# ZhenlongYuan/TSAR-MVS

Measured on AMD Instinct MI355X. Metric: depthmap Mpixels/sec (ETH3D full-res, 8 iters), higher is better.
Workload: dtype f32

## Files before the change

include/tsar.h:

```cpp
#ifndef TSAR_H_
#define TSAR_H_

#include <stddef.h>
#include <stdint.h>

#ifdef __cplusplus
extern "C" {
#endif

#define TSAR_MAX_VIEWS 64
#define TSAR_MAXCOST 2.0f

#define TSAR_OK 0
#define TSAR_ERR_INVALID (-1)
#define TSAR_ERR_HIP (-2)
#define TSAR_ERR_STATE (-3)
#define TSAR_ERR_NOMEM (-4)

#define TSAR_MEM_HOST 0
#define TSAR_MEM_DEVICE 1

#define TSAR_COMB_ALL 0
#define TSAR_COMB_BEST_N 1
#define TSAR_COMB_ANGLE 2
// ... 196 lines not shown
void tsar_device_free(int device, void* p);
int tsar_device_write(int device, void* dst, const void* host_src, size_t bytes);
int tsar_peer_copy(int dst_device, void* dst, int src_device, const void* src, size_t bytes);

int tsar_enable_kernel_timing(tsar_ctx* ctx, int enable);
int tsar_reset_kernel_timing(tsar_ctx* ctx);
int tsar_get_kernel_timing(tsar_ctx* ctx, tsar_kernel_timing* out, int cap, int* n_out);

int tsar_selftest_sqrt(tsar_ctx* ctx, int mode, uint64_t seed, uint64_t* mismatches_out);
int tsar_selftest_divide(tsar_ctx* ctx, const float* X, const float* Y, const float* Z, size_t n, float* u_out, float* v_out, int ieee);
int tsar_selftest_divide_random(tsar_ctx* ctx, int log2_triples, uint64_t seed, int mode, int guarded, uint64_t* mismatches_out,
                                uint64_t* outside_guard_out);
int tsar_selftest_sweep_census(tsar_ctx* ctx, int colour, uint64_t* out8);
int tsar_selftest_sweep_repeat(tsar_ctx* ctx, int colour, void* memo_dev, uint64_t* out8);
int tsar_selftest_prune_census(tsar_ctx* ctx, int on, uint32_t* out32);
int tsar_selftest_slic_stage(tsar_ctx* ctx, int stage, int w, int h, int mw, int mh, const tsar_slic_settings* s, const void* in0,
                             const void* in1, void* inout);

#ifdef __cplusplus
}
#endif
#endif
```

tsar-mvs_amd/api.py:

```python
from __future__ import annotations

import ctypes as C
import os

import numpy as np

_HERE = os.path.dirname(os.path.abspath(__file__))
LIB_PATH = os.environ.get("TSAR_LIB") or os.path.join(_HERE, "libtsar_hip.so")

TSAR_OK = 0
TSAR_ERR_INVALID, TSAR_ERR_HIP, TSAR_ERR_STATE, TSAR_ERR_NOMEM = -1, -2, -3, -4
MEM_HOST, MEM_DEVICE = 0, 1
COMB_ALL, COMB_BEST_N, COMB_ANGLE, COMB_GOOD = 0, 1, 2, 3
FLAG_FIX_DOWN_FAR_SEED, FLAG_FIX_RIGHT_FAR_CMP, FLAG_STRICT_DIV = 1, 2, 4
FLAG_FIX_PLANE_FIT = 8
FLAG_NO_LINE_CLOSING = 16
FLAG_TEX_FILTER_8BIT = 32
FLAG_FIX_INIT_RADIUS = 64
MAXCOST = 2.0
MAX_VIEWS = 64


class TsarError(RuntimeError):
    def __init__(self, code, msg):
# ... 57 lines not shown
    "tsar_pm_init", "tsar_pm_iterate", "tsar_pm_iterate_final", "tsar_pm_sweep", "tsar_set_sweep_counter", "tsar_pm_cost_planes", "tsar_set_plane", "tsar_get_plane",
    "tsar_load_planes", "tsar_compute_disp", "tsar_compute_disp_final", "tsar_depth_to_plane", "tsar_get_result",
    "tsar_pyramid_views", "tsar_upsample_planes", "tsar_compute_disp_final_upsampled", "tsar_get_view_image",
    "tsar_set_geom_depths", "tsar_clear_geom", "tsar_pm_rescore", "tsar_get_geom_matrices",
    "tsar_geom_pyramid", "tsar_pyramid_planes", "tsar_upsample_merge",
    "tsar_default_geom_check_params", "tsar_geom_check",
    "tsar_default_geom_reproject_params", "tsar_geom_reproject", "tsar_pm_merge_depths",
    "tsar_default_plane_prior_params", "tsar_set_plane_prior", "tsar_clear_plane_prior", "tsar_get_plane_prior",
    "tsar_default_plane_prior_build_params", "tsar_build_plane_prior",
    "tsar_set_reliable_mask", "tsar_get_reliable_mask", "tsar_lrdiff", "tsar_getview", "tsar_wmf", "tsar_set_regions", "tsar_detect_weak_texture", "tsar_ransac_regions",
    "tsar_set_region_planes", "tsar_fake_depth", "tsar_fill_textureless",
    "tsar_default_slic_settings", "tsar_slic", "tsar_default_fusion_params", "tsar_fuse", "tsar_fuse_ctx",
    "tsar_default_cloud_distance_params", "tsar_cloud_distance_ctx", "tsar_cloud_distance",
    "tsar_default_cloud_voxels_params", "tsar_cloud_voxels_ctx", "tsar_cloud_voxels",
    "tsar_host_alloc", "tsar_host_free", "tsar_device_alloc", "tsar_device_free", "tsar_device_write", "tsar_peer_copy", "tsar_enable_kernel_timing", "tsar_reset_kernel_timing", "tsar_get_kernel_timing",
    "tsar_selftest_divide", "tsar_selftest_divide_random", "tsar_selftest_sqrt", "tsar_selftest_sweep_census", "tsar_selftest_prune_census", "tsar_selftest_sweep_repeat", "tsar_selftest_slic_stage",
]

_lib = None


def load_library(path: str = LIB_PATH):
    global _lib
    if _lib is not None:
        return _lib
    if not os.path.exists(path):
        raise ImportError(f"{path} not found: build it with `make -C tsar-mvs_amd/csrc` "
                          "(or __graft_entry__.build()); there is no CPU fallback")
    L = C.CDLL(path)
    L.tsar_last_error.restype = C.c_char_p
    L.tsar_last_error.argtypes = [C.c_void_p]
# ... 84 lines not shown
    if hasattr(L, "tsar_cloud_voxels_ctx"):
        L.tsar_default_cloud_voxels_params.restype = None
        L.tsar_default_cloud_voxels_params.argtypes = [C.POINTER(CloudVoxelsParams)]
        L.tsar_cloud_voxels.argtypes = [C.c_int, C.c_void_p, C.c_int64, C.c_int, C.POINTER(CloudVoxelsParams), C.c_void_p, C.c_int, C.c_void_p, C.c_void_p, C.c_int64,
                                        C.c_void_p, C.c_void_p, C.c_void_p, C.POINTER(C.c_int64), C.POINTER(C.c_int64), C.c_int]
        L.tsar_cloud_voxels_ctx.argtypes = [C.c_void_p] + list(L.tsar_cloud_voxels.argtypes[1:])
    L.tsar_get_stream.argtypes = [C.c_void_p, C.POINTER(C.c_void_p)]
    L.tsar_synchronize.argtypes = [C.c_void_p]
    L.tsar_enable_kernel_timing.argtypes = [C.c_void_p, C.c_int]
    L.tsar_reset_kernel_timing.argtypes = [C.c_void_p]
    L.tsar_get_kernel_timing.argtypes = [C.c_void_p, C.POINTER(KernelTiming), C.c_int, C.POINTER(C.c_int)]
    L.tsar_selftest_divide.argtypes = [C.c_void_p, C.c_void_p, C.c_void_p, C.c_void_p, C.c_size_t, C.c_void_p, C.c_void_p, C.c_int]
    L.tsar_selftest_sweep_census.argtypes = [C.c_void_p, C.c_int, C.POINTER(C.c_uint64)]
    if hasattr(L, "tsar_selftest_prune_census"):
        L.tsar_selftest_prune_census.argtypes = [C.c_void_p, C.c_int, C.POINTER(C.c_uint32)]
    L.tsar_selftest_sweep_repeat.argtypes = [C.c_void_p, C.c_int, C.c_void_p, C.POINTER(C.c_uint64)]
    L.tsar_selftest_sqrt.argtypes = [C.c_void_p, C.c_int, C.c_uint64, C.POINTER(C.c_uint64)]
    L.tsar_selftest_divide_random.argtypes = [C.c_void_p, C.c_int, C.c_uint64, C.c_int, C.c_int, C.POINTER(C.c_uint64), C.POINTER(C.c_uint64)]
    L.tsar_selftest_slic_stage.argtypes = [C.c_void_p, C.c_int, C.c_int, C.c_int, C.c_int, C.c_int, C.POINTER(SlicSettings), C.c_void_p, C.c_void_p, C.c_void_p]
    _lib = L
    return L


def default_params(**kw) -> Params:
    p = Params()
    load_library().tsar_default_params(C.byref(p))
    for k, v in kw.items():
        setattr(p, k, v)
    return p

# ... 346 lines not shown
        return bad.value

    def selftest_sweep_census(self, colour: int) -> dict:
        out = (C.c_uint64 * 8)()
        self._chk(self.L.tsar_selftest_sweep_census(self._ctx, colour, out))
        keys = ("waves", "arms_any_lane", "max_lane_survivors", "max_lane_survivors_nodup", "lane_survivors", "lane_survivors_nodup", "pixels", "arms_present")
        return dict(zip(keys, [int(v) for v in out]))

    def selftest_prune_census(self, on: bool):
        if on:
            self._chk(self.L.tsar_selftest_prune_census(self._ctx, 1, None))
            return None
        out = (C.c_uint32 * 32)()
        self._chk(self.L.tsar_selftest_prune_census(self._ctx, 0, out))
        return np.array(out, np.int64).reshape(8, 4)

    def selftest_divide_random(self, log2_triples: int, seed: int, mode: int, guarded: bool = True):
        bad, out = C.c_uint64(0), C.c_uint64(0)
        self._chk(self.L.tsar_selftest_divide_random(self._ctx, log2_triples, seed, mode, int(guarded), C.byref(bad), C.byref(out)))
        return bad.value, out.value

    def _slic_stage(self, stage, w, h, mw, mh, settings, in0, in1, inout):
        p1 = _ptr(in1)[0] if in1 is not None else None
        self._chk(self.L.tsar_selftest_slic_stage(self._ctx, stage, w, h, mw, mh, C.byref(settings), _ptr(in0)[0], p1, _ptr(inout)[0]))
        return inout

    def slic_convert(self, bgra, color_space=0):
        img = np.ascontiguousarray(bgra, np.uint8).reshape(-1, 4)
        return self._slic_stage(0, img.shape[0], 1, 0, 0, SlicSettings(20, 0, 5.0, 0, color_space), img, None, np.zeros((img.shape[0], 4), np.float32))

# ... 484 lines not shown
```

tsar-mvs_amd/csrc/pm_core.h:

```cpp
#pragma once
#include <type_traits>

#include "tsar_device_math.h"

#define PM_BLOCK 256
#define PM_RW 32

#include "pm_tap_common.h"

template <bool QUAD, bool DIFF = false>
DEVFN float sample_bilinear(const DevView& vw, int w, int h, int qpitch, float u, float v, bool q8 = false) {
    u = fminf(fmaxf(u, -1.0f), (float)w);
    v = fminf(fmaxf(v, -1.0f), (float)h);
    const float fu = floorf(u), fv = floorf(v);
    float ax = u - fu, ay = v - fv;
    if (q8) { ax = rintf(ax * 256.0f) * 0.00390625f; ay = rintf(ay * 256.0f) * 0.00390625f; }
    const int iu = (int)fu, iv = (int)fv;
    float t00, t10, t01, t11;
    if (QUAD) {
        const uint32_t off = (uint32_t)(__mul24(iv + 1, qpitch) + iu + 1) * 4u;
        const uint32_t q = *(global_u32_ptr)((const char __attribute__((address_space(1)))*)vw.quad + off);
        t00 = (float)(q & 0xffu);
        t10 = (float)((q >> 8) & 0xffu);
        t01 = (float)((q >> 16) & 0xffu);
// ... 132 lines not shown
    if (pp == nullptr) return c;
    typedef float prior_entry __attribute__((ext_vector_type(4)));
    const prior_entry q = ((const __attribute__((address_space(1))) prior_entry*)pp)[y * sc->w + x];
    const float Dp = q.w;
    const float a = fabsf(D - Dp);
    const float rel = a / Dp;
    const float dclip = sc->prior_depth_clip, nclip = sc->prior_normal_clip;
    const float r_d = rel < dclip ? rel / dclip : 1.0f;
    const float s = 1.0f - ((n4.x * q.x + n4.y * q.y) + n4.z * q.z);
    const float s0 = s < 0.0f ? 0.0f : s;
    const float r_n = s < nclip ? s0 / nclip : 1.0f;
    const float t = (sc->prior_weight_depth * r_d) + (sc->prior_weight_normal * r_n);
    return Dp > 0.0f ? c + t : c;
}

template <int NB, int HR, bool STRICT, bool QUAD, int V = 0, int BLK = PM_BLOCK>
DEVFN float multiview_cost(const DevScene* __restrict__ sc, const typename TileOf<QUAD>::type* tile, int tw, int own, const float* wts, const PixelRef& pr,
                           int x, int y, const float4& n4, int& beview, float& ratio, bool prune = false, float cost_now = 0.0f, int* skipped = nullptr) {
    constexpr bool GEOM = (V & TSAR_V_GEOM) != 0;
    constexpr bool PRUNE = (V & TSAR_V_PRUNE) != 0;
    static_assert(!PRUNE || !GEOM, "the bound speaks of the photometric cost alone");
    constexpr bool PAIR = (V & TSAR_V_PAIR) != 0;
    static_assert(!PAIR || (!PRUNE && !GEOM), "the paired gathers exist for the plain fast box-11 kernels");
    constexpr int VT = V & ~(TSAR_V_GEOM | TSAR_V_REDRAW | TSAR_V_PRUNE | TSAR_V_PAIR);
    float best[NB];
#pragma unroll
    for (int k = 0; k < NB; k++) best[k] = __builtin_inff();
    const int num = sc->n_sel;
    int valid = 0, bv = -1;
    float cmin = __builtin_inff();
    float depth_h = 0.0f;
    if constexpr (GEOM) depth_h = plane_depth(sc->ref, n4, x, y);
    int vi_next = sc->sel[0];
    for (int i = 0; i < num; i++) {
        const int vi = vi_next;
        vi_next = sc->sel[i + 1 < num ? i + 1 : i];
        float c;
        if constexpr ((VT & TSAR_V_LUT) != 0) c = view_cost_lut<STRICT, (VT >> 11) & 7, (VT & TSAR_V_BUF) != 0 && !STRICT, (VT & TSAR_V_MIX) != 0 && !STRICT>(sc, sc->view[vi], tile, tw, own, wts, pr, x, y, n4);
        else if constexpr (QUAD && HR == 5 && r5_production_variant(VT) && PRUNE) {
            static_assert((VT & 250) == 250 && !STRICT, "pruning instantiations exist for the fast row-wise loop");
            ViewPrune vp;
            vp.on = prune; vp.skipped = false;
            vp.cost_now = cmin < cost_now ? TSAR_MAXCOST : cost_now;
            c = view_cost_r5<false, true, true, (VT & TSAR_V_BUF) != 0, (VT & TSAR_V_MIX) != 0, BLK, 0, true>(sc, sc->view[vi], tile, tw, own, wts, pr, x, y, n4, &vp);
            if (vp.skipped) *skipped += 1;
        } else if constexpr (QUAD && HR == 5 && PAIR && VT == 250) {
            static_assert(!STRICT, "the paired gathers exist for the fast row-wise loop");
            c = view_cost_r5<false, true, true, false, false, BLK, 0, false, true>(sc, sc->view[vi], tile, tw, own, wts, pr, x, y, n4);
        } else if constexpr (QUAD && HR == 5 && r5_production_variant(VT))
            c = view_cost_r5<STRICT, (VT & 128) != 0 && !STRICT, (VT & 8) != 0, (VT & TSAR_V_BUF) != 0, (VT & TSAR_V_MIX) != 0, BLK>(sc, sc->view[vi], tile, tw, own, wts, pr, x, y, n4);
#ifdef TSAR_EXPERIMENTS
        else if constexpr (QUAD && HR == 5 && PAIR && VT == (250 | 4194304))
            c = view_cost_r5<false, true, true, false, false, BLK, 3, false, true>(sc, sc->view[vi], tile, tw, own, wts, pr, x, y, n4);
        else if constexpr (QUAD && HR == 5 && r5_diag_variant(VT))
            c = view_cost_r5<false, true, true, true, true, BLK, (VT & 4194304) ? 1 : 2>(sc, sc->view[vi], tile, tw, own, wts, pr, x, y, n4);
#endif
        else {
            static_assert(VT == 0, "unknown tap-loop variant");
            c = view_cost_generic<HR, STRICT, QUAD, BLK>(sc, sc->view[vi], tile, tw, own, wts, pr, x, y, n4);
        }
// ... 3 lines not shown
        valid -= (int32_t)__float_as_uint(c - TSAR_MAXCOST) >> 31;
        if constexpr (GEOM) c = c + geom_term(sc, sc->view[vi], vi, x, y, depth_h);
        {
            const uint32_t worse = (uint32_t)((int32_t)__float_as_uint(cmin - c) >> 31);
            asm("v_bfi_b32 %0, %1, %2, %3" : "=v"(bv) : "v"(worse), "v"(bv), "s"(vi));
            cmin = vmin(cmin, c);
        }
        float v = c;
#pragma unroll
        for (int k = 0; k < NB; k++) {
            const float lo = vmin(best[k], v), hi = vmax(best[k], v);
            best[k] = lo;
            v = hi;
        }
    }
    int nb = valid;
    if (sc->cost_comb == TSAR_COMB_BEST_N) nb = min(nb, sc->n_best);
    if (nb <= 0) { beview = -1; ratio = 0.f; return TSAR_MAXCOST; }
    float cost = 0.f;
#pragma unroll
    for (int k = 0; k < NB; k++)
        if (k < nb) cost += best[k];
    cost = cost / (float)nb;
    ratio = num >= 2 ? best[0] / best[1] : 0.f;
    beview = bv;
    if constexpr (GEOM) cost = add_prior_term(sc, x, y, n4, depth_h, cost);
    return cost;
}

DEVFN void strip_tile(int t, int tiles_x, int tiles_y, int sw, int& tx, int& ty) {
// ... 20 lines not shown
```

tsar-mvs_amd/csrc/pm_sweep_impl.h:

```cpp
#pragma once
#include "pm_dispatch.h"

#define SWEEP_SMALL_IMAGE_TILES 3072

#define CAND_SAME (1 << 30)

DEVFN void select_candidates(const DevScene* __restrict__ sc, const float* __restrict__ c_same, const float* __restrict__ c_other,
                             int x, int y, int cand[8]) {
    const int col = sc->w, row = sc->h;
    const int p = y * col + x;
    const bool fix_seed = sc->flags & TSAR_FLAG_FIX_DOWN_FAR_SEED, fix_cmp = sc->flags & TSAR_FLAG_FIX_RIGHT_FAR_CMP;
    float cmin;
    int cp, cs;
#pragma unroll
    for (int k = 0; k < 8; k++) cand[k] = -1;
    if (y > 2) {
        cp = p - 3 * col; cmin = c_other[cp];
#pragma unroll
        for (int i = 1; i < 11; ++i)
            if (y > 2 + 2 * i) { const int q = p - (3 + 2 * i) * col; const float v = c_other[q]; if (v < cmin) { cmin = v; cp = q; } }
        cand[0] = cp;
    }
    if (y < row - 3) {
        cp = p + 3 * col;
// ... 70 lines not shown
    uint32_t* seq;
    uint32_t* changed;
    uint32_t launch, valid_from;
    int mode;
    int slot_off;
    int prune_steps;
    uint32_t* prune_counts;
};

template <int NB, int HR, bool STRICT, bool QUAD, int V, int BLK>
DEVFN float pruned_cost(const DevScene* __restrict__ sc, const typename TileOf<QUAD>::type* tile, int tw, int own, const float* wts, const PixelRef& pr,
                        int x, int y, const float4& n4, int& beview, float& ratio, int step, float cost_now, int prune_steps, uint32_t* prune_counts) {
    if constexpr ((V & TSAR_V_PRUNE) == 0) {
        return multiview_cost<NB, HR, STRICT, QUAD, V, BLK>(sc, tile, tw, own, wts, pr, x, y, n4, beview, ratio);
    } else {
        bool prune = step >= 0 && step < prune_steps;
        float c;
#pragma unroll 1
        for (;;) {
            int skipped = 0;
            c = multiview_cost<NB, HR, STRICT, QUAD, V, BLK>(sc, tile, tw, own, wts, pr, x, y, n4, beview, ratio, prune, cost_now, &skipped);
            const bool redo = skipped != 0 && __any(c < cost_now);
            if (prune && prune_counts != nullptr) {
                const uint64_t act = __ballot(1);
                if ((threadIdx.x & 63) == __ffsll((long long)act) - 1) {
                    uint32_t* k = prune_counts + 4 * step;
                    atomicAdd(k + 0, 1u); atomicAdd(k + 1, (uint32_t)sc->n_sel); atomicAdd(k + 2, (uint32_t)skipped); atomicAdd(k + 3, redo ? 1u : 0u);
                }
            }
            if (!redo) break;
            prune = false;
        }
        return c;
    }
}

template <int NB, int HR, bool STRICT, bool QUAD, int V = 0, int BLK = PM_BLOCK, bool CMP = false>
__global__ __launch_bounds__(BLK) void pm_sweep_kernel(const DevScene* __restrict__ sc, int colour,
                                                            const float* __restrict__ c_same, const float4* __restrict__ n_same,
                                                            const float* __restrict__ c_other, const float4* __restrict__ n_other,
                                                            float* c_out, float4* n_out, float* __restrict__ ratio_out,
                                                            int32_t* __restrict__ beview_out, uint32_t stream_id, int do_prop,
                                                            int do_refine, int tiles_x, int n_tiles, int cost_consistent, int strip_w,
                                                            const float* __restrict__ final_text, SweepMemo memo) {
    extern __shared__ __attribute__((aligned(16))) unsigned char lds_raw[];
    typedef typename TileOf<QUAD>::type TileT;
    constexpr int RW = PM_RW;
    constexpr int SWEEP_RH = 2 * BLK / RW;
    const int hr = HR > 0 ? HR : sc->hrad, vr = HR > 0 ? HR : sc->vrad;
    const int tw = RW + 2 * hr, th = SWEEP_RH + 2 * vr;
    constexpr bool LUTW = (V & TSAR_V_LUT) != 0;
    const size_t lut_bytes = LUTW ? (size_t)(sc->lut_classes + 1) * 1024 : 0;
    TileT* tile = (TileT*)(lds_raw + lut_bytes);
// ... 273 lines not shown
constexpr bool sweep_has_packed_form() { return QUAD && ((HR == 5 && r5_production_variant(V & ~(TSAR_V_GEOM | TSAR_V_PRUNE))) || (V & TSAR_V_LUT) != 0); }

template <int NB, int HR, bool STRICT, bool QUAD, int V = 0, int BLK = PM_BLOCK>
static int launch_sweep_t(tsar_ctx* ctx, int colour, const PlaneBuf& same_in, const PlaneBuf& other, const PlaneBuf& same_out,
                          uint32_t stream_id, int do_prop, int do_refine) {
    constexpr int SWEEP_RH = 2 * BLK / PM_RW;
#ifdef TSAR_EXPERIMENTS
    const size_t lds_pad = ctx->lds_pad;
#else
    constexpr size_t lds_pad = 0;
#endif
    SweepMemo memo;
    memo.cand = ctx->memo_cand; memo.seq = ctx->memo_seq; memo.changed = ctx->changed_seq;
    memo.launch = ctx->launch_seq; memo.valid_from = ctx->memo_valid_from;
    memo.mode = (ctx->memo_mode && ctx->memo_cand && ctx->cost_consistent && !ctx->final_text) ? 1 : 0;
    memo.prune_steps = ((V & TSAR_V_PRUNE) != 0 && do_refine && ctx->call_launch >= ctx->prune_from) ? ctx->prune_steps : 0;
    memo.prune_counts = (V & TSAR_V_PRUNE) != 0 ? ctx->prune_counts : nullptr;
    bool packed = false;
    if constexpr (sweep_has_packed_form<HR, QUAD, V>())
        packed = memo.mode && do_prop && ctx->compact_from >= 0 && ctx->call_launch >= ctx->compact_from;
    auto kern = pm_sweep_kernel<NB, HR, STRICT, QUAD, V, BLK, false>;
    if constexpr (sweep_has_packed_form<HR, QUAD, V>())
        if (packed) kern = pm_sweep_kernel<NB, HR, STRICT, QUAD, V, BLK, true>;
    const size_t slots = packed ? 6 * (size_t)BLK : 0;
    TapGrid g;
    if (const int rc = tap_grid(ctx, kern, SWEEP_RH, BLK, QUAD, V, lds_pad + slots, g)) return rc;
    memo.slot_off = packed ? (int)(g.lds - slots) : 0;
    {
        ScopedKernelTimer tm(ctx, (V & TSAR_V_GEOM) ? "pm_sweep_geom" : "pm_sweep");
        ScopedKernelTimer tm_packed(ctx, packed ? "pm_sweep_packed" : nullptr);
        ScopedKernelTimer tm_prune(ctx, (V & TSAR_V_PRUNE) ? "pm_sweep_prune" : nullptr);
// ... 16 lines not shown
```

tsar-mvs_amd/csrc/pm_tap_common.h:

```cpp
#pragma once

typedef const uint32_t __attribute__((address_space(1)))* global_u32_ptr;
typedef const float __attribute__((address_space(1)))* global_f32_ptr;

template <bool STRICT, bool ROW = false>
DEVFN void tap_line_base(const float* H, float a, float& bx, float& by, float& bz) {
    bx = STRICT ? H[0] * a : fma_(H[ROW ? 1 : 0], a, H[2]);
    by = STRICT ? H[3] * a : fma_(H[ROW ? 4 : 3], a, H[5]);
    bz = STRICT ? H[6] * a : fma_(H[ROW ? 7 : 6], a, H[8]);
}
template <bool STRICT, bool ROW = false>
DEVFN void tap_homogeneous(const float* H, float t, float bx, float by, float bz, float& X, float& Y, float& Z) {
    X = fma_(H[ROW ? 0 : 1], t, bx); Y = fma_(H[ROW ? 3 : 4], t, by); Z = fma_(H[ROW ? 6 : 7], t, bz);
    if (STRICT) { X += H[2]; Y += H[5]; Z += H[8]; }
}
DEVFN void pixel_homogeneous(const float* H, float xi, float yj, float& X, float& Y, float& Z) {
    float bx, by, bz;
    tap_line_base<false>(H, xi, bx, by, bz);
    tap_homogeneous<false>(H, yj, bx, by, bz, X, Y, Z);
}

template <bool STRICT, bool GUARD>
DEVFN void tap_divide(float X, float Y, float Z, float& u, float& v) {
    if (STRICT) {
// ... 109 lines not shown
    bool textured;
};
DEVFN PixelRef pixel_ref_from_sums(float sum_ref, float sum_ref_ref, float inv_wsum) {
    PixelRef pr;
    pr.inv_wsum = inv_wsum;
    sum_ref *= pr.inv_wsum;
    sum_ref_ref *= pr.inv_wsum;
    pr.mean_ref = sum_ref;
    pr.var_ref = sum_ref_ref - sum_ref * sum_ref;
    pr.textured = !(pr.var_ref < 1e-5f);
    return pr;
}

struct ViewPrune {
    float cost_now;
    bool on;
    bool skipped;
};
#define PM_PRUNE_E 0.9f
#define PM_PRUNE_EA 0.45f
#define PM_PRUNE_SLACK 1.0e-4f
DEVFN bool prune_proven(const TapSums& t, float aw, float ar, float arr, const PixelRef& pr, float cost_now) {
    const float E = PM_PRUNE_EA * aw * aw;
    const float a_lo = fma_(aw, arr, -(ar * ar)) - E;
    const float b_lo = fma_(aw, t.src_src, -(t.src * t.src)) - E;
    const float c_hi = fabsf(fma_(aw, t.ref_src, -(ar * t.src))) + E;
    const float raw = __builtin_amdgcn_rcpf(aw);
    const float q = fma_(-(c_hi * c_hi), __builtin_amdgcn_rcpf(b_lo), a_lo) * raw;
    const float vs = (b_lo * raw) * pr.inv_wsum, vr = pr.var_ref - PM_PRUNE_E;
    const float n2 = fma_(-q, pr.inv_wsum * __builtin_amdgcn_rcpf(pr.var_ref + PM_PRUNE_E), 1.0f);
    const float eg = PM_PRUNE_E * __builtin_amdgcn_rsqf(vr * vs);
    const float tt = 1.0f - cost_now;
// ... 16 lines not shown
```

tsar-mvs_amd/csrc/pm_tap_r5.h:

```cpp
#pragma once

#define PM_PRUNE_FIRST_LINE 2
#define PM_PRUNE_LAST_LINE 4

template <bool STRICT, bool ROW, bool D16, bool BUF, bool MIX, int BLK, int DIAG = 0, bool PRUNE = false, bool PAIR = false>
DEVFN float view_cost_r5(const DevScene* __restrict__ sc, const DevView& vw, const unsigned short* tile, int tw, int own, const float* wts,
                         const PixelRef& pr, int x, int y, const float4& n4, ViewPrune* vp = nullptr) {
    static_assert(!(STRICT && ROW), "the row-wise walk changes the summation order: fast mode only");
    static_assert(!PRUNE || (ROW && D16 && !STRICT && DIAG == 0), "the partial-window bound is written for the fast row-wise loop");
    static_assert(!MIX || (BUF && !STRICT), "the half-float difference texture serves the fast arithmetic's blend through buffer loads");
    static_assert(!PAIR || (ROW && D16 && !STRICT && !BUF && !MIX && !PRUNE), "the paired gathers are written for the plain fast row-wise loop on the byte texture");
    static_assert(DIAG != 3 || PAIR, "DIAG 3 is a form of the paired loop");
    const int w = sc->w, h = sc->h, qp = sc->quad_pitch;
    const int qorg = quad_border_bytes(qp);
    float H[9];
    if (STRICT) plane_homography(sc->ref, vw, n4, H, sc->k_sparse != 0);
    else plane_homography_fast(sc->ref, vw, n4, H);
    float sum_src = 0.f, sum_src_src = 0.f, sum_ref_src = 0.f;
    bool need_clamp;
    if (!STRICT) {
        float Xc, Yc, Zc;
        pixel_homogeneous(H, (float)x, (float)y, Xc, Yc, Zc);
        const float a = fabsf(H[0]) + fabsf(H[1]), b = fabsf(H[3]) + fabsf(H[4]), c = fabsf(H[6]) + fabsf(H[7]);
        const float Zmin = fma_(-5.0f, c, Zc);
// ... 124 lines not shown
            if (MIX) s = blend_dquad(q2[jj], ax[jj], ay[jj]);
            else s = blend_quad<!STRICT>(q[jj], ax[jj], ay[jj]);
            if (jj == 0 && DIAG != 2) {
                if (D16)
                    asm("s_waitcnt lgkmcnt(0)" : "+v"(rcol[0]), "+v"(rcol[1]), "+v"(rcol[2]), "+v"(rcol[3]), "+v"(rcol[4]), "+v"(rcol[5]),
                        "+v"(wcol[0]), "+v"(wcol[1]), "+v"(wcol[2]), "+v"(s));
                else
                    asm("s_waitcnt lgkmcnt(0)" : "+v"(wcol[0]), "+v"(wcol[1]), "+v"(wcol[2]), "+v"(s));
            }
            const float r = D16 ? rcol[jj] : tile_value(ROW ? tile[own + i * tw + (2 * jj - 5)] : tile[own + (2 * jj - 5) * tw + i]);
            const float wt = wcol[jj >> 1][jj & 1];
            const TapSums t = tap_accumulate<STRICT>(TapSums{sum_src, sum_src_src, sum_ref_src}, wt, r, s);
            sum_src = t.src; sum_src_src = t.src_src; sum_ref_src = t.ref_src;
        }
    };
    auto pruned = [&](int line) {
        if constexpr (PRUNE) {
            if (vp->on && line >= PM_PRUNE_FIRST_LINE - 1 && line < PM_PRUNE_LAST_LINE) {
                float pa_w = 0.f, pa_r = 0.f, pa_rr = 0.f;
#pragma unroll 1
                for (int l = 0; l <= line; l++) {
#pragma unroll
                    for (int jj = 0; jj < 6; jj++) {
                        const float wt = wts[(6 * jj + l) * BLK], r = tile_value(tile[own + (2 * l - 5) * tw + (2 * jj - 5)]);
                        const float wr = wt * r;
                        pa_w += wt;
                        pa_r += wr;
                        pa_rr = fma_(wr, r, pa_rr);
                    }
                }
                if (__all(prune_proven(TapSums{sum_src, sum_src_src, sum_ref_src}, pa_w, pa_r, pa_rr, pr, vp->cost_now))) { vp->skipped = true; return true; }
            }
        }
        return false;
    };
    if (need_clamp) {
#pragma unroll 1
        for (int i = -5; i <= 5; i += 2) { line6(i, std::true_type(), std::false_type()); if (pruned((i + 5) >> 1)) return TSAR_MAXCOST; }
    } else if (MIX && !(PRUNE && vp->on)) {
#pragma unroll
        for (int i = -5; i <= 5; i += 2) line6(i, std::false_type(), std::bool_constant<MIX>());
    } else {
#pragma unroll 1
        for (int i = -5; i <= 5; i += 2) { line6(i, std::false_type(), std::false_type()); if (pruned((i + 5) >> 1)) return TSAR_MAXCOST; }
    }
    return ncc_cost(pr, TapSums{sum_src, sum_src_src, sum_ref_src});
}

__host__ __device__ constexpr bool r5_diag_variant(int V) { return V == (250 | TSAR_V_BUF | TSAR_V_MIX | 4194304) || V == (250 | TSAR_V_BUF | TSAR_V_MIX | 8388608); }
__host__ __device__ constexpr bool r5_production_variant(int V) { return V == 114 || V == 122 || V == 250 || V == (114 | TSAR_V_BUF) || V == (122 | TSAR_V_BUF) || V == (250 | TSAR_V_BUF) || V == (250 | TSAR_V_BUF | TSAR_V_MIX); }
```

tsar-mvs_amd/csrc/tsar_api.hip:

```cpp
#include <float.h>
#include <math.h>
#include <stdio.h>
#include <stdlib.h>
#include <string.h>

#include <algorithm>

#include "tsar_dev.h"

ScopedKernelTimer::ScopedKernelTimer(tsar_ctx* c, const char* name) : ctx(c) {
    if (!ctx->timing || !name) return;
    for (size_t k = 0; k < ctx->timers.size(); k++)
        if (ctx->timers[k].name == name) ti = (int)k;
    if (ti < 0) {
        ctx->timers.emplace_back();
        ctx->timers.back().name = name;
        ti = (int)ctx->timers.size() - 1;
    }
    if (hipEventCreate(&e0) != hipSuccess) { ti = -1; return; }
    if (hipEventCreate(&e1) != hipSuccess) { hipEventDestroy(e0); ti = -1; return; }
    hipEventRecord(e0, ctx->stream);
}
ScopedKernelTimer::~ScopedKernelTimer() {
    if (ti < 0) return;
// ... 166 lines not shown

static void read_knobs(tsar_ctx* ctx) {
    auto num = [](const char* name, int dflt) { const char* e = getenv(name); return e && e[0] ? atoi(e) : dflt; };
    auto on = [](const char* name, bool dflt) { const char* e = getenv(name); return e && e[0] ? e[0] != '0' : dflt; };
    ctx->variant = num("TSAR_VARIANT", ctx->variant);
    ctx->buffer_gather = on("TSAR_BUFFER_GATHER", true);
    ctx->mix_gather = on("TSAR_MIX_GATHER", true);
    ctx->strip_w = num("TSAR_STRIP", -1);
    ctx->buffer_from = num("TSAR_BUFFER_FROM", 1);
    ctx->force_block = num("TSAR_BLOCK", 0);
    ctx->memo_mode = num("TSAR_MEMO", 1);
    ctx->compact_from = num("TSAR_COMPACT_FROM", 6);
    ctx->prune = num("TSAR_PRUNE", 1);
    ctx->prune_steps = std::min(std::max(num("TSAR_PRUNE_STEPS", 2), 0), 8);
    ctx->prune_from = num("TSAR_PRUNE_FROM", 1);
    ctx->pair = num("TSAR_PAIR", 3);
    ctx->lut_mode = num("TSAR_LUT", 1);
    ctx->ransac_wgs = num("TSAR_RANSAC_WGS", 8);
    ctx->ransac_chain = num("TSAR_RANSAC_CHAIN", 8);
    ctx->ransac_lookahead = num("TSAR_RANSAC_LOOKAHEAD", 0);
    ctx->ransac_poll_limit = num("TSAR_RANSAC_POLL_LIMIT", 1 << 15);
    ctx->ransac_cooperative = on("TSAR_RANSAC_COOPERATIVE", true);
    ctx->ransac_force_fallback = on("TSAR_RANSAC_FORCE_FALLBACK", false);
    ctx->trace_host = getenv("TSAR_TRACE_HOST") != nullptr;
#ifdef TSAR_EXPERIMENTS
    ctx->lds_pad = (size_t)num("TSAR_LDS_PAD", 0);
#endif
}

extern "C" int tsar_create(int device, tsar_ctx** out) {
// ... 26 lines not shown
    for (auto& p : ctx->geom_maps) dev_free(p);
    ctx->geom_maps.clear();
    for (auto& p : ctx->hscene.geom_depth) p = nullptr;
    ctx->hscene.geom_on = 0;
}
static void free_prior(tsar_ctx* ctx) {
    dev_free(ctx->prior);
    ctx->hscene.prior = nullptr;
}
static void free_planes(tsar_ctx* ctx) {
    for (int b = 0; b < 2; b++) { dev_free(ctx->buf[b].c); dev_free(ctx->buf[b].n4); }
    dev_free(ctx->ratio); dev_free(ctx->depth); dev_free(ctx->scale); dev_free(ctx->lrdiff); dev_free(ctx->confid);
    dev_free(ctx->fakedepth); dev_free(ctx->beview); dev_free(ctx->canny); dev_free(ctx->out4);
    dev_free(ctx->memo_cand); dev_free(ctx->memo_seq); dev_free(ctx->changed_seq);
    if (ctx->prune_counts) { (void)hipFree(ctx->prune_counts); ctx->prune_counts = nullptr; }
    dev_free(ctx->resize4);
    ctx->have_resize = false;
}

extern "C" int tsar_destroy(tsar_ctx* ctx) {
    if (!ctx) return TSAR_OK;
    (void)enter_ctx(ctx);
    if (ctx->stream) hipStreamSynchronize(ctx->stream);
    drain_timers(ctx);
    free_views(ctx);
    free_planes(ctx);
    free_geom(ctx);
    free_prior(ctx);
    dev_free(ctx->dscene); dev_free(ctx->region_text); dev_free(ctx->region_size); dev_free(ctx->region_n4);
    if (ctx->scratch.base) hipFree(ctx->scratch.base);
// ... 1107 lines not shown
int launch_sweep_repeat(tsar_ctx* ctx, int colour, unsigned long long* memo, unsigned long long* dout);
extern "C" int tsar_selftest_sweep_repeat(tsar_ctx* ctx, int colour, void* memo_dev, uint64_t* out8) {
    CHECK_CTX(ctx);
    if (!memo_dev || !out8) return fail(ctx, TSAR_ERR_INVALID, "memo_dev / out8 is NULL");
    NEED_VIEWS(ctx);
    NEED_STATE(ctx);
    return run_counters(ctx, 8, out8, [&](unsigned long long* dc) { return launch_sweep_repeat(ctx, colour & 1, (unsigned long long*)memo_dev, dc); });
}
extern "C" int tsar_selftest_sweep_census(tsar_ctx* ctx, int colour, uint64_t* out8) {
    CHECK_CTX(ctx);
    NEED_VIEWS(ctx);
    NEED_STATE(ctx);
    if (!out8) return fail(ctx, TSAR_ERR_INVALID, "out8 is NULL");
    return run_counters(ctx, 8, out8, [&](unsigned long long* dc) { return launch_sweep_census(ctx, colour & 1, dc); });
}
extern "C" int tsar_selftest_prune_census(tsar_ctx* ctx, int on, uint32_t* out32) {
    CHECK_CTX(ctx);
    TSAR_HIP_TRY(ctx, hipStreamSynchronize(ctx->stream));
    if (on) {
        if (!ctx->prune_counts) TSAR_HIP_TRY(ctx, hipMalloc((void**)&ctx->prune_counts, 32 * sizeof(uint32_t)));
        TSAR_HIP_TRY(ctx, hipMemset(ctx->prune_counts, 0, 32 * sizeof(uint32_t)));
        return TSAR_OK;
    }
    if (!ctx->prune_counts) return fail(ctx, TSAR_ERR_INVALID, "no prune census is running");
    if (out32) TSAR_HIP_TRY(ctx, hipMemcpy(out32, ctx->prune_counts, 32 * sizeof(uint32_t), hipMemcpyDeviceToHost));
    TSAR_HIP_TRY(ctx, hipFree(ctx->prune_counts));
    ctx->prune_counts = nullptr;
    return TSAR_OK;
}
```

tsar-mvs_amd/csrc/tsar_dev.h:

```cpp
#pragma once
#include <hip/hip_runtime.h>
#include <stdint.h>
#include <stdio.h>
#include <stdlib.h>

#include <chrono>
#include <string>
#include <vector>

#include "../../include/tsar.h"

#define TSAR_LUT_LINES 32
#define TSAR_LUT_TAPS 40
#define TSAR_LUT_MAX_CLASSES 144
#define TSAR_MAX_SELECTED 32

struct DevView {
    float K[9];
    float R[9];
    float t[3];
    float t_abs_lo;
    float A[9];
    float b[3];
    float t_abs_hi;
// ... 92 lines not shown
    float4* region_n4 = nullptr;
    int exact_sqrt_probe = 0;
    int exact_div_probe = 0;
    int sweeps_done = 0;
    int32_t* memo_cand = nullptr;
    uint32_t* memo_seq = nullptr;
    uint32_t* changed_seq = nullptr;
    uint32_t launch_seq = 0;
    uint32_t memo_valid_from = 1;
    int call_launch = 0;
    int memo_mode = 1;
    int compact_from = 6;
    int prune = 1;
    int prune_steps = 2;
    int prune_from = 1;
    int pair = 3;
    uint32_t* prune_counts = nullptr;
    std::vector<tsar_camera> cams;
    bool views_u8 = false;
    float4* resize4 = nullptr;
    bool have_resize = false;
    const float* final_text = nullptr;
    std::vector<float*> geom_maps;
    float4* prior = nullptr;
    int variant = 2;
    bool mix_gather = true;
    bool buffer_gather = true;
    int strip_w = -1;
    int buffer_from = 1;
    int force_block = 0;
    int lut_mode = 1;
    int ransac_wgs = 8;
// ... 253 lines not shown
```

Before: 51.43.

## Let proven-dead lanes skip view cost work and redo only when pruned lanes win

Per-lane pruning now marks a lane as dead once its bound proves it cannot beat the current cost, and later lines skip the tap accumulation for dead lanes even when the whole wave cannot leave. The number of views pruned at each line and the count of dead lanes are packed into bitfields. A redo is triggered only when a lane that improved actually had dead views, instead of whenever any view was skipped. A waves-per-EU occupancy hint is also added to the compact prune kernel. Alongside this, a per-line prune census selftest API is added. The tradeoffs are more divergence and more register pressure in the inner loop.

New measurement: 51.89, median of 6. No clear change (+0.9%).

```diff
diff --git a/include/tsar.h b/include/tsar.h
--- a/include/tsar.h
+++ b/include/tsar.h
@@ -234,6 +234,7 @@
 int tsar_selftest_sweep_census(tsar_ctx* ctx, int colour, uint64_t* out8);
 int tsar_selftest_sweep_repeat(tsar_ctx* ctx, int colour, void* memo_dev, uint64_t* out8);
 int tsar_selftest_prune_census(tsar_ctx* ctx, int on, uint32_t* out32);
+int tsar_selftest_prune_census_lines(tsar_ctx* ctx, int on, uint64_t* out128);
 int tsar_selftest_slic_stage(tsar_ctx* ctx, int stage, int w, int h, int mw, int mh, const tsar_slic_settings* s, const void* in0,
                              const void* in1, void* inout);
 
diff --git a/tsar-mvs_amd/api.py b/tsar-mvs_amd/api.py
--- a/tsar-mvs_amd/api.py
+++ b/tsar-mvs_amd/api.py
@@ -95,7 +95,7 @@
     "tsar_default_cloud_distance_params", "tsar_cloud_distance_ctx", "tsar_cloud_distance",
     "tsar_default_cloud_voxels_params", "tsar_cloud_voxels_ctx", "tsar_cloud_voxels",
     "tsar_host_alloc", "tsar_host_free", "tsar_device_alloc", "tsar_device_free", "tsar_device_write", "tsar_peer_copy", "tsar_enable_kernel_timing", "tsar_reset_kernel_timing", "tsar_get_kernel_timing",
-    "tsar_selftest_divide", "tsar_selftest_divide_random", "tsar_selftest_sqrt", "tsar_selftest_sweep_census", "tsar_selftest_prune_census", "tsar_selftest_sweep_repeat", "tsar_selftest_slic_stage",
+    "tsar_selftest_divide", "tsar_selftest_divide_random", "tsar_selftest_sqrt", "tsar_selftest_sweep_census", "tsar_selftest_prune_census", "tsar_selftest_prune_census_lines", "tsar_selftest_sweep_repeat", "tsar_selftest_slic_stage",
 ]
 
 _lib = None
@@ -210,6 +210,8 @@
     L.tsar_selftest_sweep_census.argtypes = [C.c_void_p, C.c_int, C.POINTER(C.c_uint64)]
     if hasattr(L, "tsar_selftest_prune_census"):
         L.tsar_selftest_prune_census.argtypes = [C.c_void_p, C.c_int, C.POINTER(C.c_uint32)]
+    if hasattr(L, "tsar_selftest_prune_census_lines"):
+        L.tsar_selftest_prune_census_lines.argtypes = [C.c_void_p, C.c_int, C.POINTER(C.c_uint64)]
     L.tsar_selftest_sweep_repeat.argtypes = [C.c_void_p, C.c_int, C.c_void_p, C.POINTER(C.c_uint64)]
     L.tsar_selftest_sqrt.argtypes = [C.c_void_p, C.c_int, C.c_uint64, C.POINTER(C.c_uint64)]
     L.tsar_selftest_divide_random.argtypes = [C.c_void_p, C.c_int, C.c_uint64, C.c_int, C.c_int, C.POINTER(C.c_uint64), C.POINTER(C.c_uint64)]
@@ -586,6 +588,14 @@
         out = (C.c_uint32 * 32)()
         self._chk(self.L.tsar_selftest_prune_census(self._ctx, 0, out))
         return np.array(out, np.int64).reshape(8, 4)
+
+    def selftest_prune_census_lines(self, on: bool):
+        if on:
+            self._chk(self.L.tsar_selftest_prune_census_lines(self._ctx, 1, None))
+            return None
+        out = (C.c_uint64 * 128)()
+        self._chk(self.L.tsar_selftest_prune_census_lines(self._ctx, 0, out))
+        return np.array(out, np.uint64).astype(np.int64).reshape(8, 16)
 
     def selftest_divide_random(self, log2_triples: int, seed: int, mode: int, guarded: bool = True):
         bad, out = C.c_uint64(0), C.c_uint64(0)
diff --git a/tsar-mvs_amd/csrc/pm_core.h b/tsar-mvs_amd/csrc/pm_core.h
--- a/tsar-mvs_amd/csrc/pm_core.h
+++ b/tsar-mvs_amd/csrc/pm_core.h
@@ -170,9 +170,13 @@
     return Dp > 0.0f ? c + t : c;
 }
 
+struct MultiviewPrune {
+    uint32_t left = 0;
+    uint32_t died = 0;
+};
 template <int NB, int HR, bool STRICT, bool QUAD, int V = 0, int BLK = PM_BLOCK>
 DEVFN float multiview_cost(const DevScene* __restrict__ sc, const typename TileOf<QUAD>::type* tile, int tw, int own, const float* wts, const PixelRef& pr,
-                           int x, int y, const float4& n4, int& beview, float& ratio, bool prune = false, float cost_now = 0.0f, int* skipped = nullptr) {
+                           int x, int y, const float4& n4, int& beview, float& ratio, int prune = 0, float cost_now = 0.0f, MultiviewPrune* pv = nullptr) {
     constexpr bool GEOM = (V & TSAR_V_GEOM) != 0;
     constexpr bool PRUNE = (V & TSAR_V_PRUNE) != 0;
     static_assert(!PRUNE || !GEOM, "the bound speaks of the photometric cost alone");
@@ -199,7 +203,13 @@
             vp.on = prune; vp.skipped = false;
             vp.cost_now = cmin < cost_now ? TSAR_MAXCOST : cost_now;
             c = view_cost_r5<false, true, true, (VT & TSAR_V_BUF) != 0, (VT & TSAR_V_MIX) != 0, BLK, 0, true>(sc, sc->view[vi], tile, tw, own, wts, pr, x, y, n4, &vp);
-            if (vp.skipped) *skipped += 1;
+            if (vp.skipped) pv->left += 1u << (8 * (vp.skipped - 1));
+            static_assert(PM_PRUNED_COST == 4.0f && TSAR_MAXCOST == 2.0f && TSAR_MAX_SELECTED < 256, "the bit tests below");
+            if (prune) {
+                const uint32_t gone = (__float_as_uint(c) + 0x3f800000u) >> 31;
+                const uint32_t sh = (__float_as_uint(c) >> 18) & 24u;
+                valid += (int32_t)(gone << sh);
+            }
         } else if constexpr (QUAD && HR == 5 && PAIR && VT == 250) {
             static_assert(!STRICT, "the paired gathers exist for the fast row-wise loop");
             c = view_cost_r5<false, true, true, false, false, BLK, 0, false, true>(sc, sc->view[vi], tile, tw, own, wts, pr, x, y, n4);
@@ -233,6 +243,7 @@
             v = hi;
         }
     }
+    if constexpr (PRUNE) { pv->died = (uint32_t)valid >> 8; valid &= 0xff; }
     int nb = valid;
     if (sc->cost_comb == TSAR_COMB_BEST_N) nb = min(nb, sc->n_best);
     if (nb <= 0) { beview = -1; ratio = 0.f; return TSAR_MAXCOST; }
diff --git a/tsar-mvs_amd/csrc/pm_sweep_impl.h b/tsar-mvs_amd/csrc/pm_sweep_impl.h
--- a/tsar-mvs_amd/csrc/pm_sweep_impl.h
+++ b/tsar-mvs_amd/csrc/pm_sweep_impl.h
@@ -108,29 +108,55 @@
     if constexpr ((V & TSAR_V_PRUNE) == 0) {
         return multiview_cost<NB, HR, STRICT, QUAD, V, BLK>(sc, tile, tw, own, wts, pr, x, y, n4, beview, ratio);
     } else {
-        bool prune = step >= 0 && step < prune_steps;
+        int prune = step >= 0 && step < (prune_steps & 255) ? 1 + (prune_steps >> 8) : 0;
         float c;
 #pragma unroll 1
         for (;;) {
-            int skipped = 0;
-            c = multiview_cost<NB, HR, STRICT, QUAD, V, BLK>(sc, tile, tw, own, wts, pr, x, y, n4, beview, ratio, prune, cost_now, &skipped);
-            const bool redo = skipped != 0 && __any(c < cost_now);
+            MultiviewPrune pv;
+            c = multiview_cost<NB, HR, STRICT, QUAD, V, BLK>(sc, tile, tw, own, wts, pr, x, y, n4, beview, ratio, prune, cost_now, &pv);
+            const int skipped = (int)((pv.left & 255u) + ((pv.left >> 8) & 255u) + (pv.left >> 16));
+            bool redo = __any(c < cost_now && pv.died != 0);
+#ifdef TSAR_EXPERIMENTS
+            if (prune > 2) redo = false;
+#endif
             if (prune && prune_counts != nullptr) {
                 const uint64_t act = __ballot(1);
-                if ((threadIdx.x & 63) == __ffsll((long long)act) - 1) {
+                const bool first = (threadIdx.x & 63) == __ffsll((long long)act) - 1;
+                if (first) {
                     uint32_t* k = prune_counts + 4 * step;
                     atomicAdd(k + 0, 1u); atomicAdd(k + 1, (uint32_t)sc->n_sel); atomicAdd(k + 2, (uint32_t)skipped); atomicAdd(k + 3, redo ? 1u : 0u);
                 }
+                if (unsigned long long* kl = *(unsigned long long* const*)(prune_counts + 32)) {
+                    kl += 16 * step;
+                    const uint32_t n_act = (uint32_t)__popcll(act), views = (uint32_t)sc->n_sel;
+                    uint32_t entering = views, gone_before = 0, dead_sum = 0;
+#pragma unroll 1
+                    for (int j = 0; j < 3; j++) {
+                        const uint32_t left_j = (pv.left >> (8 * j)) & 255u;
+                        uint32_t died_j = 0;
+#pragma unroll 1
+                        for (int b = 0; b < 6; b++) died_j += (uint32_t)__popcll(__ballot((pv.died >> (8 * j + b)) & 1u)) << b;
+                        if (first) {
+                            atomicAdd(kl + 4 * j + 0, (unsigned long long)entering); atomicAdd(kl + 4 * j + 1, (unsigned long long)left_j);
+                            atomicAdd(kl + 4 * j + 2, (unsigned long long)(n_act * views - gone_before)); atomicAdd(kl + 4 * j + 3, prune > 1 ? (unsigned long long)died_j : 0ull);
+                        }
+                        entering -= left_j; gone_before += died_j; dead_sum += died_j;
+                    }
+                    if (first) {
+                        atomicAdd(kl + 12, redo ? 1ull : 0ull); atomicAdd(kl + 13, redo && skipped == 0 ? 1ull : 0ull);
+                        atomicAdd(kl + 14, (unsigned long long)(dead_sum - n_act * (uint32_t)skipped)); atomicAdd(kl + 15, (unsigned long long)(n_act * (views - (uint32_t)skipped)));
+                    }
+                }
             }
             if (!redo) break;
-            prune = false;
+            prune = 0;
         }
         return c;
     }
 }
 
 template <int NB, int HR, bool STRICT, bool QUAD, int V = 0, int BLK = PM_BLOCK, bool CMP = false>
-__global__ __launch_bounds__(BLK) void pm_sweep_kernel(const DevScene* __restrict__ sc, int colour,
+__global__ __launch_bounds__(BLK) __attribute__((amdgpu_waves_per_eu((V & TSAR_V_PRUNE) != 0 && CMP ? 4 : 1))) void pm_sweep_kernel(const DevScene* __restrict__ sc, int colour,
                                                             const float* __restrict__ c_same, const float4* __restrict__ n_same,
                                                             const float* __restrict__ c_other, const float4* __restrict__ n_other,
                                                             float* c_out, float4* n_out, float* __restrict__ ratio_out,
@@ -434,7 +460,7 @@
     memo.cand = ctx->memo_cand; memo.seq = ctx->memo_seq; memo.changed = ctx->changed_seq;
     memo.launch = ctx->launch_seq; memo.valid_from = ctx->memo_valid_from;
     memo.mode = (ctx->memo_mode && ctx->memo_cand && ctx->cost_consistent && !ctx->final_text) ? 1 : 0;
-    memo.prune_steps = ((V & TSAR_V_PRUNE) != 0 && do_refine && ctx->call_launch >= ctx->prune_from) ? ctx->prune_steps : 0;
+    memo.prune_steps = ((V & TSAR_V_PRUNE) != 0 && do_refine && ctx->call_launch >= ctx->prune_from) ? (ctx->prune_steps | (ctx->prune_lanes << 8)) : 0;
     memo.prune_counts = (V & TSAR_V_PRUNE) != 0 ? ctx->prune_counts : nullptr;
     bool packed = false;
     if constexpr (sweep_has_packed_form<HR, QUAD, V>())
diff --git a/tsar-mvs_amd/csrc/pm_tap_common.h b/tsar-mvs_amd/csrc/pm_tap_common.h
--- a/tsar-mvs_amd/csrc/pm_tap_common.h
+++ b/tsar-mvs_amd/csrc/pm_tap_common.h
@@ -147,8 +147,8 @@
 
 struct ViewPrune {
     float cost_now;
-    bool on;
-    bool skipped;
+    int on;
+    int skipped;
 };
 #define PM_PRUNE_E 0.9f
 #define PM_PRUNE_EA 0.45f
diff --git a/tsar-mvs_amd/csrc/pm_tap_r5.h b/tsar-mvs_amd/csrc/pm_tap_r5.h
--- a/tsar-mvs_amd/csrc/pm_tap_r5.h
+++ b/tsar-mvs_amd/csrc/pm_tap_r5.h
@@ -2,6 +2,7 @@
 
 #define PM_PRUNE_FIRST_LINE 2
 #define PM_PRUNE_LAST_LINE 4
+#define PM_PRUNED_COST 4.0f
 
 template <bool STRICT, bool ROW, bool D16, bool BUF, bool MIX, int BLK, int DIAG = 0, bool PRUNE = false, bool PAIR = false>
 DEVFN float view_cost_r5(const DevScene* __restrict__ sc, const DevView& vw, const unsigned short* tile, int tw, int own, const float* wts,
@@ -162,37 +163,60 @@
             sum_src = t.src; sum_src_src = t.src_src; sum_ref_src = t.ref_src;
         }
     };
+    auto dead = [&]() { return PRUNE && vp->cost_now < 0.0f; };
     auto pruned = [&](int line) {
         if constexpr (PRUNE) {
             if (vp->on && line >= PM_PRUNE_FIRST_LINE - 1 && line < PM_PRUNE_LAST_LINE) {
-                float pa_w = 0.f, pa_r = 0.f, pa_rr = 0.f;
+                const bool was_dead = dead();
+                bool proven = false;
+                if (!was_dead) {
+                    float pa_w = 0.f, pa_r = 0.f, pa_rr = 0.f;
 #pragma unroll 1
-                for (int l = 0; l <= line; l++) {
-#pragma unroll
-                    for (int jj = 0; jj < 6; jj++) {
-                        const float wt = wts[(6 * jj + l) * BLK], r = tile_value(tile[own + (2 * l - 5) * tw + (2 * jj - 5)]);
-                        const float wr = wt * r;
-                        pa_w += wt;
-                        pa_r += wr;
-                        pa_rr = fma_(wr, r, pa_rr);
+                    for (int l = 0; l <= line; l++) {
+#pragma unroll
+                        for (int jj = 0; jj < 6; jj++) {
+                            const float wt = wts[(6 * jj + l) * BLK], r = tile_value(tile[own + (2 * l - 5) * tw + (2 * jj - 5)]);
+                            const float wr = wt * r;
+                            pa_w += wt;
+                            pa_r += wr;
+                            pa_rr = fma_(wr, r, pa_rr);
+                        }
                     }
+                    proven = prune_proven(TapSums{sum_src, sum_src_src, sum_ref_src}, pa_w, pa_r, pa_rr, pr, vp->cost_now);
                 }
-                if (__all(prune_proven(TapSums{sum_src, sum_src_src, sum_ref_src}, pa_w, pa_r, pa_rr, pr, vp->cost_now))) { vp->skipped = true; return true; }
+#ifdef TSAR_EXPERIMENTS
+                if (vp->on > 2) proven = true;
+#endif
+                const bool leave = __all(was_dead || proven);
+                if (proven && (leave || vp->on > 1)) vp->cost_now = (float)(PM_PRUNE_FIRST_LINE - 2 - line);
+                if (leave) { vp->skipped = line - (PM_PRUNE_FIRST_LINE - 2); return true; }
             }
         }
         return false;
     };
     if (need_clamp) {
 #pragma unroll 1
-        for (int i = -5; i <= 5; i += 2) { line6(i, std::true_type(), std::false_type()); if (pruned((i + 5) >> 1)) return TSAR_MAXCOST; }
+        for (int i = -5; i <= 5; i += 2) {
+            if constexpr (PRUNE) { if (!dead()) line6(i, std::true_type(), std::false_type()); }
+            else line6(i, std::true_type(), std::false_type());
+            if (pruned((i + 5) >> 1)) return PM_PRUNED_COST - vp->cost_now;
+        }
     } else if (MIX && !(PRUNE && vp->on)) {
 #pragma unroll
         for (int i = -5; i <= 5; i += 2) line6(i, std::false_type(), std::bool_constant<MIX>());
     } else {
 #pragma unroll 1
-        for (int i = -5; i <= 5; i += 2) { line6(i, std::false_type(), std::false_type()); if (pruned((i + 5) >> 1)) return TSAR_MAXCOST; }
+        for (int i = -5; i <= 5; i += 2) {
+            if constexpr (PRUNE) { if (!dead()) line6(i, std::false_type(), std::false_type()); }
+            else line6(i, std::false_type(), std::false_type());
+            if (pruned((i + 5) >> 1)) return PM_PRUNED_COST - vp->cost_now;
+        }
     }
-    return ncc_cost(pr, TapSums{sum_src, sum_src_src, sum_ref_src});
+    if constexpr (PRUNE) {
+        const float c = ncc_cost(pr, TapSums{sum_src, sum_src_src, sum_ref_src});
+        if (vp->on > 1) return dead() ? PM_PRUNED_COST - vp->cost_now : c;
+        return c;
+    } else return ncc_cost(pr, TapSums{sum_src, sum_src_src, sum_ref_src});
 }
 
 __host__ __device__ constexpr bool r5_diag_variant(int V) { return V == (250 | TSAR_V_BUF | TSAR_V_MIX | 4194304) || V == (250 | TSAR_V_BUF | TSAR_V_MIX | 8388608); }
diff --git a/tsar-mvs_amd/csrc/tsar_api.hip b/tsar-mvs_amd/csrc/tsar_api.hip
--- a/tsar-mvs_amd/csrc/tsar_api.hip
+++ b/tsar-mvs_amd/csrc/tsar_api.hip
@@ -204,6 +204,10 @@
     ctx->prune = num("TSAR_PRUNE", 1);
     ctx->prune_steps = std::min(std::max(num("TSAR_PRUNE_STEPS", 2), 0), 8);
     ctx->prune_from = num("TSAR_PRUNE_FROM", 1);
+    ctx->prune_lanes = num("TSAR_PRUNE_LANES", 1) != 0;
+#ifdef TSAR_EXPERIMENTS
+    if (num("TSAR_PRUNE_LANES", 1) == 2) ctx->prune_lanes = 2;
+#endif
     ctx->pair = num("TSAR_PAIR", 3);
     ctx->lut_mode = num("TSAR_LUT", 1);
     ctx->ransac_wgs = num("TSAR_RANSAC_WGS", 8);
@@ -260,6 +264,7 @@
     dev_free(ctx->fakedepth); dev_free(ctx->beview); dev_free(ctx->canny); dev_free(ctx->out4);
     dev_free(ctx->memo_cand); dev_free(ctx->memo_seq); dev_free(ctx->changed_seq);
     if (ctx->prune_counts) { (void)hipFree(ctx->prune_counts); ctx->prune_counts = nullptr; }
+    if (ctx->prune_lines) { (void)hipFree(ctx->prune_lines); ctx->prune_lines = nullptr; }
     dev_free(ctx->resize4);
     ctx->have_resize = false;
 }
@@ -1397,17 +1402,48 @@
     if (!out8) return fail(ctx, TSAR_ERR_INVALID, "out8 is NULL");
     return run_counters(ctx, 8, out8, [&](unsigned long long* dc) { return launch_sweep_census(ctx, colour & 1, dc); });
 }
-extern "C" int tsar_selftest_prune_census(tsar_ctx* ctx, int on, uint32_t* out32) {
-    CHECK_CTX(ctx);
-    TSAR_HIP_TRY(ctx, hipStreamSynchronize(ctx->stream));
-    if (on) {
-        if (!ctx->prune_counts) TSAR_HIP_TRY(ctx, hipMalloc((void**)&ctx->prune_counts, 32 * sizeof(uint32_t)));
-        TSAR_HIP_TRY(ctx, hipMemset(ctx->prune_counts, 0, 32 * sizeof(uint32_t)));
-        return TSAR_OK;
-    }
-    if (!ctx->prune_counts) return fail(ctx, TSAR_ERR_INVALID, "no prune census is running");
-    if (out32) TSAR_HIP_TRY(ctx, hipMemcpy(out32, ctx->prune_counts, 32 * sizeof(uint32_t), hipMemcpyDeviceToHost));
+static const size_t kPruneBlockBytes = 32 * sizeof(uint32_t) + sizeof(uint64_t);
+static int prune_block(tsar_ctx* ctx) {
+    if (ctx->prune_counts) return TSAR_OK;
+    TSAR_HIP_TRY(ctx, hipMalloc((void**)&ctx->prune_counts, kPruneBlockBytes));
+    TSAR_HIP_TRY(ctx, hipMemset(ctx->prune_counts, 0, kPruneBlockBytes));
+    return TSAR_OK;
+}
+static int prune_block_release(tsar_ctx* ctx) {
+    if (ctx->prune_counting || ctx->prune_lines || !ctx->prune_counts) return TSAR_OK;
     TSAR_HIP_TRY(ctx, hipFree(ctx->prune_counts));
     ctx->prune_counts = nullptr;
     return TSAR_OK;
 }
+extern "C" int tsar_selftest_prune_census(tsar_ctx* ctx, int on, uint32_t* out32) {
+    CHECK_CTX(ctx);
+    TSAR_HIP_TRY(ctx, hipStreamSynchronize(ctx->stream));
+    if (on) {
+        if (const int rc = prune_block(ctx)) return rc;
+        TSAR_HIP_TRY(ctx, hipMemset(ctx->prune_counts, 0, 32 * sizeof(uint32_t)));
+        ctx->prune_counting = true;
+        return TSAR_OK;
+    }
+    if (!ctx->prune_counting) return fail(ctx, TSAR_ERR_INVALID, "no prune census is running");
+    if (out32) TSAR_HIP_TRY(ctx, hipMemcpy(out32, ctx->prune_counts, 32 * sizeof(uint32_t), hipMemcpyDeviceToHost));
+    ctx->prune_counting = false;
+    return prune_block_release(ctx);
+}
+extern "C" int tsar_selftest_prune_census_lines(tsar_ctx* ctx, int on, uint64_t* out128) {
+    CHECK_CTX(ctx);
+    TSAR_HIP_TRY(ctx, hipStreamSynchronize(ctx->stream));
+    if (on) {
+        if (const int rc = prune_block(ctx)) return rc;
+        if (!ctx->prune_lines) TSAR_HIP_TRY(ctx, hipMalloc((void**)&ctx->prune_lines, 128 * sizeof(uint64_t)));
+        TSAR_HIP_TRY(ctx, hipMemset(ctx->prune_lines, 0, 128 * sizeof(uint64_t)));
+        const uint64_t addr = (uint64_t)(uintptr_t)ctx->prune_lines;
+        TSAR_HIP_TRY(ctx, hipMemcpy(ctx->prune_counts + 32, &addr, sizeof(addr), hipMemcpyHostToDevice));
+        return TSAR_OK;
+    }
+    if (!ctx->prune_lines) return fail(ctx, TSAR_ERR_INVALID, "no per-check prune census is running");
+    if (out128) TSAR_HIP_TRY(ctx, hipMemcpy(out128, ctx->prune_lines, 128 * sizeof(uint64_t), hipMemcpyDeviceToHost));
+    TSAR_HIP_TRY(ctx, hipMemset(ctx->prune_counts + 32, 0, sizeof(uint64_t)));
+    TSAR_HIP_TRY(ctx, hipFree(ctx->prune_lines));
+    ctx->prune_lines = nullptr;
+    return prune_block_release(ctx);
+}
diff --git a/tsar-mvs_amd/csrc/tsar_dev.h b/tsar-mvs_amd/csrc/tsar_dev.h
--- a/tsar-mvs_amd/csrc/tsar_dev.h
+++ b/tsar-mvs_amd/csrc/tsar_dev.h
@@ -130,8 +130,11 @@
     int prune = 1;
     int prune_steps = 2;
     int prune_from = 1;
+    int prune_lanes = 1;
+    unsigned long long* prune_lines = nullptr;
     int pair = 3;
     uint32_t* prune_counts = nullptr;
+    bool prune_counting = false;
     std::vector<tsar_camera> cams;
     bool views_u8 = false;
     float4* resize4 = nullptr;
```
